# maxsonate/video-diffusion-nnx

Hardware: AMD Instinct MI355X
Metric: denoised frames/sec, 16fx64x64 1000-step DDPM (higher is better)
Workload: dtype bf16; 1 GPU; config_v2_2 (north-star shape): Unet3D dim=64 C=1, 16f x 64x64, DDPM T=1000 p_sample_loop (UNet forward + p_sample per step, hipGraph replay); value = n_gpus*B*F/(T*s_per_step); batch_per_gpu=64, parallelism=dp1 (independent samples, no collective), mfma_operands=bf16, storage=weights fp32 master, activations bf16, fp32 accumulate, process_group=none (single process)

## Files before the change

video_diffusion_nnx_amd/csrc/sla.hip:

```cpp
#include "vdx_common.h"
#include "vdx_internal.h"
#include <stdlib.h>

namespace vdx {

constexpr int SLA_PART = 32 * 32 + 64;

template <int MODE>
__global__ __launch_bounds__(256) void sla_ctx_kernel(const SlaArgs P) {
    using M = Mma<MODE>;
    constexpr int KT = M::KT, KC = M::KC, RS = ROW_STRIDE;
    constexpr int APIECES = KT / 4;
    constexpr int NCHN = 64 / KC;
    constexpr int RSE = NCHN * 64 + 16;

    extern __shared__ __attribute__((aligned(16))) char smem[];
    float* m_run = reinterpret_cast<float*>(smem);
    float* s_run = m_run + 32;
    float* alpha = s_run + 32;
    float* pm = alpha + 32;
    char* xs = smem + 1024;
    char* ws = xs + 64 * RS;
    char* eT = ws + 64 * RS;
    char* vT = eT + 32 * RSE;
// ... 301 lines not shown
#pragma unroll
    for (int tmo = 0; tmo < TMO; ++tmo) {
        const int co = (w * TMO + tmo) * 16 + 4 * q;
        if (co >= P.C) continue;
#pragma unroll
        for (int tn = 0; tn < 4; ++tn) {
            const int row = r0 + tn * 16 + lp;
            if (row >= P.N) continue;
            const float4 xr = load4_f32_or_bf16(P.x, xbase + (size_t)row * P.C + co, P.io_bf16);
            float4 v;
            v.x = oacc[tmo][tn][0] + xr.x; v.y = oacc[tmo][tn][1] + xr.y;
            v.z = oacc[tmo][tn][2] + xr.z; v.w = oacc[tmo][tn][3] + xr.w;
            store4_f32_or_bf16(P.y, xbase + (size_t)row * P.C + co, v, P.io_bf16);
        }
    }
}


template <int MODE, int NKT, bool IO16>
struct SlaTile {
    using M = Mma<MODE>;
    static_assert(!IO16 || MODE == MODE_BF16, "bf16 activation storage implies bf16 MFMA operands");
    static constexpr int PCH = IO16 ? 8 : 4;
    static constexpr int APIECES = M::KT / PCH;
    static constexpr int XP = 64 * APIECES * NKT / 512;
    static constexpr int PLANE = 64 * ROW_STRIDE;
    static constexpr int BUF = NKT * PLANE;
    float4 xpre[XP];
    __device__ __forceinline__ void fetch(const float* x, size_t xbase, int io_bf16, int r0, int N, int C, int tid) {
#pragma unroll
        for (int u = 0; u < XP; ++u) {
            const int i = tid + 512 * u;
            const int kt = i / (64 * APIECES), rem = i % (64 * APIECES);
            const int row = rem / APIECES, c = kt * M::KT + (rem % APIECES) * PCH;
            xpre[u] = make_float4(0.f, 0.f, 0.f, 0.f);
            if (r0 + row < N && c < C) {
                if (IO16) xpre[u] = *reinterpret_cast<const float4*>(reinterpret_cast<const char*>(x) + (xbase + (size_t)(r0 + row) * C + c) * 2);
                else xpre[u] = load4_f32_or_bf16(x, xbase + (size_t)(r0 + row) * C + c, io_bf16);
            }
        }
    }
    __device__ __forceinline__ void put(char* xs, int tid) const {
#pragma unroll
        for (int u = 0; u < XP; ++u) {
            const int i = tid + 512 * u;
            const int kt = i / (64 * APIECES), rem = i % (64 * APIECES);
            char* dst = xs + kt * PLANE + (rem / APIECES) * ROW_STRIDE;
            if (IO16) *reinterpret_cast<float4*>(dst + (rem % APIECES) * 16) = xpre[u];
            else M::store4(dst, (rem % APIECES) * 4, xpre[u]);
        }
    }
};

template <bool FULL>
__device__ __forceinline__ void ctx8_softmax_step(f32x4 (&acc)[2][4], float (&m_run)[2], float (&s_run)[2], f32x4 (&cacc)[2][2], int nleft) {
    constexpr float L2E = 1.44269504088896f;
#pragma unroll
    for (int dt = 0; dt < 2; ++dt) {
        if (!FULL) {
#pragma unroll
            for (int tn = 0; tn < 2; ++tn)
#pragma unroll
                for (int r = 0; r < 4; ++r) if (tn * 16 + r >= nleft) acc[tn][dt][r] = -1e30f;
        }
        float mx = fmaxf(fmaxf(fmaxf(acc[0][dt][0], acc[0][dt][1]), fmaxf(acc[0][dt][2], acc[0][dt][3])),
                         fmaxf(fmaxf(acc[1][dt][0], acc[1][dt][1]), fmaxf(acc[1][dt][2], acc[1][dt][3])));
        mx = max_q(mx);
        const float mn = fmaxf(m_run[dt], mx);
        const float alpha = __builtin_amdgcn_exp2f((m_run[dt] - mn) * L2E);
        m_run[dt] = mn;
        const float nb = -mn * L2E;
        float ssum = 0.f;
#pragma unroll
        for (int tn = 0; tn < 2; ++tn)
#pragma unroll
            for (int r = 0; r < 4; ++r) {
                float e = __builtin_amdgcn_exp2f(__builtin_fmaf(acc[tn][dt][r], L2E, nb));
                if (!FULL) e = (tn * 16 + r >= nleft) ? 0.f : e;
                acc[tn][dt][r] = e;
                ssum += e;
            }
        s_run[dt] = s_run[dt] * alpha + reduce_q(ssum);
#pragma unroll
        for (int et = 0; et < 2; ++et)
#pragma unroll
            for (int r = 0; r < 4; ++r) cacc[et][dt][r] *= alpha;
    }
}

template <int MODE, int NKT, bool IO16>
__global__ __launch_bounds__(512) void sla_ctx8_kernel(const SlaArgs P) {
    using M = Mma<MODE>;
    using T = SlaTile<MODE, NKT, IO16>;
    constexpr int RS = ROW_STRIDE;
    extern __shared__ __attribute__((aligned(16))) char smem[];
    const int tid = threadIdx.x, lane = tid & 63, h = tid >> 6;
    const int lp = lane & 15, q = lane >> 4;
    const int n = blockIdx.x / P.nchunk, chunk = blockIdx.x % P.nchunk;
    const int R = P.nsub * 64;
    const size_t xbase = (size_t)n * P.N * P.C;

    uint4 wf[NKT][2][4];
#pragma unroll
    for (int kt = 0; kt < NKT; ++kt)
#pragma unroll
        for (int ch = 0; ch < 2; ++ch)
#pragma unroll
            for (int tm = 0; tm < 4; ++tm) {
                const char* base = reinterpret_cast<const char*>(tm < 2 ? P.wk : P.wv);
                wf[kt][ch][tm] = *reinterpret_cast<const uint4*>(base + ((size_t)(h * 32 + (tm & 1) * 16 + lp) * P.CPad + kt * M::KT) * M::ES + ch * 64 + q * 16);
            }
    float m_run[2] = {-1e30f, -1e30f}, s_run[2] = {0.f, 0.f};
    f32x4 cacc[2][2];
#pragma unroll
    for (int i = 0; i < 2; ++i) { cacc[i][0] = f32x4{0.f, 0.f, 0.f, 0.f}; cacc[i][1] = f32x4{0.f, 0.f, 0.f, 0.f}; }

    T t;
    t.fetch(P.x, xbase, P.io_bf16, chunk * R, P.N, P.C, tid);
    t.put(smem, tid);
    __syncthreads();
    for (int sub = 0; sub < P.nsub; ++sub) {
        const int r0 = chunk * R + sub * 64;
        if (r0 >= P.N) break;
        const char* xs = smem + (sub & 1) * T::BUF;
        const bool more = (sub + 1 < P.nsub) && (r0 + 64 < P.N);
        if (more) t.fetch(P.x, xbase, P.io_bf16, r0 + 64, P.N, P.C, tid);
#pragma unroll
        for (int hf = 0; hf < 2; ++hf) {
            f32x4 acc[2][4];
#pragma unroll
            for (int i = 0; i < 2; ++i)
#pragma unroll
                for (int j = 0; j < 4; ++j) acc[i][j] = f32x4{0.f, 0.f, 0.f, 0.f};
#pragma unroll
            for (int kt = 0; kt < NKT; ++kt)
#pragma unroll
                for (int ch = 0; ch < 2; ++ch) {
                    uint4 xa[2];
#pragma unroll
                    for (int tn = 0; tn < 2; ++tn)
                        xa[tn] = *reinterpret_cast<const uint4*>(xs + kt * T::PLANE + ((hf * 2 + tn) * 16 + lp) * RS + ch * 64 + q * 16);
#pragma unroll
                    for (int tn = 0; tn < 2; ++tn)
#pragma unroll
                        for (int tm = 0; tm < 4; ++tm) M::mma(acc[tn][tm], xa[tn], wf[kt][ch][tm]);
                }
            if (r0 + 64 <= P.N) ctx8_softmax_step<true>(acc, m_run, s_run, cacc, 0);
            else ctx8_softmax_step<false>(acc, m_run, s_run, cacc, P.N - (r0 + hf * 32 + 4 * q));
#pragma unroll
            for (int tn = 0; tn < 2; ++tn)
#pragma unroll
                for (int et = 0; et < 2; ++et)
#pragma unroll
                    for (int dt = 0; dt < 2; ++dt) M::mma16(cacc[et][dt], acc[tn][2 + et], acc[tn][dt]);
        }
        if (more) t.put(smem + ((sub + 1) & 1) * T::BUF, tid);
        __syncthreads();
    }
    if (P.nchunk == 1) {
        char* ct = reinterpret_cast<char*>(P.ctxT) + (size_t)(n * P.heads + h) * 32 * 32 * M::ES;
#pragma unroll
        for (int dt = 0; dt < 2; ++dt) {
            const float inv = 1.0f / s_run[dt];
#pragma unroll
            for (int et = 0; et < 2; ++et)
#pragma unroll
                for (int r = 0; r < 4; ++r) M::store1(ct + (size_t)(et * 16 + 4 * q + r) * 32 * M::ES, dt * 16 + lp, cacc[et][dt][r] * inv);
        }
        return;
    }
    float* part = P.part + ((size_t)(n * P.nchunk + chunk) * P.heads + h) * SLA_PART;
#pragma unroll
    for (int et = 0; et < 2; ++et)
#pragma unroll
        for (int dt = 0; dt < 2; ++dt)
            *reinterpret_cast<float4*>(part + (dt * 16 + lp) * 32 + et * 16 + 4 * q) =
                make_float4(cacc[et][dt][0], cacc[et][dt][1], cacc[et][dt][2], cacc[et][dt][3]);
    if (q == 0) {
#pragma unroll
        for (int dt = 0; dt < 2; ++dt) { part[1024 + dt * 16 + lp] = m_run[dt]; part[1056 + dt * 16 + lp] = s_run[dt]; }
    }
}

template <int MODE, int NKT, int TMO, int TNO, bool IO16>
__global__ __launch_bounds__(512, NKT == 1 ? 4 : 2) void sla_out8_kernel(const SlaArgs P) {
    using M = Mma<MODE>;
    using T = SlaTile<MODE, NKT, IO16>;
    constexpr int RS = ROW_STRIDE, KC = M::KC, HD = 256;
    constexpr int RSO = HD * M::ES + 16;
    constexpr int NCHO = HD / KC;
    constexpr bool WO_RES = (TMO * NCHO <= 16);

    extern __shared__ __attribute__((aligned(16))) char smem[];
    char* os = smem + 2 * T::BUF;
    constexpr int RSY = NKT * M::KT * 4 + 16;
    char* ys = os + 64 * RSO;
    const int tid = threadIdx.x, lane = tid & 63, h = tid >> 6;
    const int lp = lane & 15, q = lane >> 4;
    const int n = blockIdx.x / P.nchunk, chunk = blockIdx.x % P.nchunk;
    const int R = P.nsub * 64;
    const size_t xbase = (size_t)n * P.N * P.C;

    uint4 wqf[NKT][2][2];
#pragma unroll
    for (int kt = 0; kt < NKT; ++kt)
#pragma unroll
        for (int ch = 0; ch < 2; ++ch)
#pragma unroll
            for (int tm = 0; tm < 2; ++tm)
                wqf[kt][ch][tm] = *reinterpret_cast<const uint4*>(reinterpret_cast<const char*>(P.wq) +
                    ((size_t)(h * 32 + tm * 16 + lp) * P.CPad + kt * M::KT) * M::ES + ch * 64 + q * 16);
// ... 634 lines not shown
```

video_diffusion_nnx_amd/csrc/conv_igemm.hip:

```cpp
#include "vdx_common.h"
#include <type_traits>
#include "vdx_internal.h"
#include "vdx_glds.h"
#include "model.h"
#include <stdlib.h>
#include <string.h>

namespace vdx {

typedef unsigned u32x4 __attribute__((ext_vector_type(4)));
typedef unsigned u32x2 __attribute__((ext_vector_type(2)));
constexpr unsigned OOB = 0xFFFFFFF0u;

template <int MODE, int BC, int TN, int NW, int INF>
__global__ __launch_bounds__(64 * NW, (NW == 8 && TN == 2) ? 4 : 2) void conv_igemm_kernel(const ConvArgs P) {
    using M = Mma<MODE>;
    constexpr int KT = M::KT;
    constexpr int RS = ROW_STRIDE;
    constexpr int WAVES_C = BC / 64;
    constexpr int WAVES_P = NW / WAVES_C;
    constexpr int NT = 64 * NW;
    constexpr int TM = 4;
    constexpr int APIECES = KT / 4;
    constexpr int WREGS = BC * 8 / NT;
// ... 1354 lines not shown
    const int taps = a.kind ? 16 : a.kh * a.kw;
    const double ho = a.kind ? 2.0 * a.H : (a.H + a.stride - 1) / a.stride, wo = a.kind ? 2.0 * a.W : (a.W + a.stride - 1) / a.stride;
    const double cin = a.C0 + a.C1;
    w.flops = 2.0 * a.NF * ho * wo * cin * a.Cout * (a.kind ? 4 : taps);
    w.bytes = (double)a.NF * a.H * a.W * (a.C0 * (a.x0_bf16 ? 2.0 : 4.0) + a.C1 * (a.x1_bf16 ? 2.0 : 4.0)) + a.NF * ho * wo * a.Cout * (a.y_bf16 ? 2.0 : 4.0)
            + (a.res ? a.NF * ho * wo * a.Cout * (a.res_bf16 ? 2.0 : 4.0) : 0.0) + es * taps * cin * a.Cout;
    snprintf(w.shape, sizeof(w.shape), "%s%dx%d %d->%d %dx%dx%d%s%s%s%s", a.kind ? "convT" : "conv", a.kind ? 4 : a.kh, a.kind ? 4 : a.kw, a.C0 + a.C1, a.Cout,
             a.NF, a.H, a.W, a.stride == 2 ? " s2" : "", a.pro ? " +prologue" : "", a.res ? " +res" : "", a.C1 ? " concat" : "");
    return w;
}
}

static bool tiles16_3x3(int mode, const ConvArgs& a) {
    return mode == MODE_BF16 && a.kind == 0 && a.kh == 3 && a.kw == 3 && a.stride == 1 && a.H % 16 == 0 && a.W % 16 == 0 &&
           (long)a.NF * (a.H / 16) * (a.W / 16) >= 1024;
}
static bool conv64_shape(int mode, const ConvArgs& a) {
    return tiles16_3x3(mode, a) && a.C0 == 64 && a.C1 == 0 && a.Cout == 64 && a.wrows >= 64 && a.wrow0 >= 0 && a.wrow0 + 64 <= a.wrows &&
           (!a.res || (!a.pro && a.x0_bf16 && !a.res_bf16)) && (size_t)a.NF * a.H * a.W * 64 * (a.y_bf16 ? 2 : 4) < 0xFFFFFFF0ull &&
           (!a.pro || (a.groups <= 32 && 64 % a.groups == 0)) && (!a.out_stats || (a.out_groups <= 32 && 64 % a.out_groups == 0));
}
static bool conv64q_pro_eligible(int mode, const ConvArgs& a) { return conv64_shape(mode, a) && a.x0_bf16 && a.pro; }
static bool conv64r_eligible(int mode, const ConvArgs& a) { return conv64_shape(mode, a) && a.x0_bf16 && !a.pro && !a.res; }
static bool conv64d_eligible(int mode, const ConvArgs& a) { return conv64_shape(mode, a) && a.x0_bf16 && !a.pro && a.res; }
static bool conv64p_eligible(int mode, const ConvArgs& a) { return conv64_shape(mode, a) && !a.x0_bf16; }
static bool conv64p_c32_eligible(int mode, const ConvArgs& a) {
    return tiles16_3x3(mode, a) && a.C0 == 32 && a.C1 == 0 && a.Cout == 32 && a.wrows == 32 && a.wrow0 == 0 && a.CinPad == 64 && a.x0_bf16 &&
           a.y_bf16 && !a.res && (!a.pro || (a.groups <= 32 && 32 % a.groups == 0)) && (!a.out_stats || (a.out_groups <= 32 && 32 % a.out_groups == 0));
}
static bool conv64q_cout32_eligible(int mode, const ConvArgs& a) {
    return tiles16_3x3(mode, a) && a.Cout == 32 && a.x0_bf16 && a.x1_bf16 && !a.pro && a.y_bf16 && ((a.C0 == 32 && a.C1 == 32) || (a.C0 == 64 && a.C1 == 64)) &&
           a.CinPad == a.C0 + a.C1 && a.wrows == 32 && a.wrow0 == 0 && !a.res &&
           (!a.out_stats || (a.out_groups <= 32 && 32 % a.out_groups == 0 && (32 / a.out_groups) <= 8 && 8 % (32 / a.out_groups) == 0));
}
static bool conv64q_cin128_eligible(int mode, const ConvArgs& a) {
    return tiles16_3x3(mode, a) && a.Cout == 64 && a.x0_bf16 && (!a.C1 || a.x1_bf16) && !a.pro && ((a.C0 == 64 && a.C1 == 64) || (a.C0 == 128 && a.C1 == 0)) &&
           a.wrows == 64 && a.wrow0 == 0 && !a.res && (!a.out_stats || (a.out_groups <= 32 && 32 % (64 / a.out_groups) == 0 && 64 % a.out_groups == 0)) &&
           (long)a.NF * a.H * a.W * 256 < 0xFFFFFFF0l;
}

hipError_t launch_conv(int mode, ConvArgs a, hipStream_t st) {
    const int K = a.kind ? 2 : a.kh;
    if (a.kind) { a.stride = 1; a.Ho = a.H; a.Wo = a.W; a.Hy = 2 * a.H; a.Wy = 2 * a.W; }
    else { a.Ho = (a.H + a.stride - 1) / a.stride; a.Wo = (a.W + a.stride - 1) / a.stride; a.Hy = a.Ho; a.Wy = a.Wo; }
    a.CinPad = conv_cin_pad(mode, a.C0 + a.C1);
    const int ES = mode == MODE_F32 ? 4 : 2;
    const size_t npix = (size_t)a.NF * a.H * a.W;
    if (a.wrows <= 0) { a.wrows = a.Cout; a.wrow0 = 0; }
    const size_t b0 = npix * a.C0 * (a.x0_bf16 ? 2 : 4), b1 = npix * a.C1 * (a.x1_bf16 ? 2 : 4), bw = (size_t)(a.kind ? 16 : a.kh * a.kw) * a.wrows * a.CinPad * ES;
    if (b0 >= 0xFFFFFFF0ull || b1 >= 0xFFFFFFF0ull || bw >= 0xFFFFFFF0ull) return hipErrorInvalidValue;
    a.x0_bytes = (unsigned)b0; a.x1_bytes = (unsigned)b1; a.w_bytes = (unsigned)bw;
    if (conv3x3_ws_eligible(mode, a)) {
        const ConvWork cw = conv_work(mode, a);
        LaunchScope ls(st, "conv3x3_ws_kernel", cw.flops, cw.bytes, "<%d, %s> %s", conv3x3_ws_geo(a), a.pro ? "true" : "false", cw.shape);
        return launch_conv3x3_ws(a, st);
    }
    if (conv4x4_ws_eligible(mode, a)) {
        const ConvWork cw = conv_work(mode, a);
        LaunchScope ls(st, "conv4x4_ws_kernel", cw.flops, cw.bytes, "<%d, %d, %d> %s", a.kind == 1 ? a.H : a.H / 2, a.kind == 1 ? 2 : 1, a.Cout == 64 ? 64 : 128, cw.shape);
        return launch_conv4x4_ws(a, st);
    }
    if (resample32_eligible(mode, a)) {
        const ConvWork cw = conv_work(mode, a);
        LaunchScope ls(st, "resample32_kernel", cw.flops, cw.bytes, "<%d> %s", a.kind, cw.shape);
        return launch_resample32(a, st);
    }
    if (conv1x1_pw_eligible(mode, a)) {
        const ConvWork cw = conv_work(mode, a);
        LaunchScope ls(st, "conv1x1_pw_kernel", cw.flops, cw.bytes, "<%d> %s", conv1x1_pw_rows(a), cw.shape);
        return launch_conv1x1_pw(a, st);
    }
    if (conv64q_pro_eligible(mode, a)) {
        const ConvWork cw = conv_work(mode, a);
        LaunchScope ls(st, "conv64q_kernel", cw.flops, cw.bytes, "<cin 64, pro %d, y16 %d> %s", a.pro, a.y_bf16, cw.shape);
        return launch_conv64q(a, st);
    }
    if (conv64r_eligible(mode, a)) {
        const ConvWork cw = conv_work(mode, a);
        LaunchScope ls(st, "conv64r_kernel", cw.flops, cw.bytes, "<pro 0, y16 %d> %s", a.y_bf16, cw.shape);
        return launch_conv64r(a, st);
    }
    if (conv64d_eligible(mode, a)) {
        const ConvWork cw = conv_work(mode, a);
        LaunchScope ls(st, "conv64d_kernel", cw.flops, cw.bytes, "<x16 %d, pro %d, y16 %d, res %d> %s", a.x0_bf16, a.pro, a.y_bf16, a.res ? 1 : 0, cw.shape);
        return launch_conv64d(a, st);
    }
    if (conv64p_eligible(mode, a)) {
        const ConvWork cw = conv_work(mode, a);
        LaunchScope ls(st, "conv64p_kernel", cw.flops, cw.bytes, "<x16 %d, pro %d, y16 %d, res %d> %s", a.x0_bf16, a.pro, a.y_bf16, a.res ? 1 : 0, cw.shape);
        return launch_conv64p(a, st);
    }
    if (conv64p_c32_eligible(mode, a)) {
        const ConvWork cw = conv_work(mode, a);
        LaunchScope ls(st, "conv64p_kernel", cw.flops, cw.bytes, "<x16 1, pro %d, y16 1, res 0, C 32> %s", a.pro, cw.shape);
        return launch_conv64p(a, st);
    }
    if (conv64q_cout32_eligible(mode, a)) {
        const ConvWork cw = conv_work(mode, a);
        LaunchScope ls(st, "conv64q_kernel", cw.flops, cw.bytes, "<cin %d, pro 0, y16 1, cout 32> %s", a.C0 + a.C1, cw.shape);
        return launch_conv64q(a, st);
    }
    if (conv64q_cin128_eligible(mode, a)) {
        const ConvWork cw = conv_work(mode, a);
        LaunchScope ls(st, "conv64q_kernel", cw.flops, cw.bytes, "<cin 128, pro 0, y16 %d> %s", a.y_bf16, cw.shape);
        return launch_conv64q(a, st);
    }
    const int BC = a.Cout <= 64 ? 64 : 128;
// ... 46 lines not shown
```

video_diffusion_nnx_amd/csrc/conv_ws.hip:

```cpp
#include "vdx_common.h"
#include "vdx_internal.h"
#include "vdx_glds.h"
#include <type_traits>

namespace vdx {

namespace {

__device__ __attribute__((aligned(16))) unsigned g_zero_page[4];

__device__ __forceinline__ int frag_off(int row, int key, int q) { return row * 128 + (((q ^ (key & 3)) | (key & 4)) << 4); }

constexpr int WS_SLAB = 128 * 128;
constexpr int WS_STORES = 16;

}

constexpr int WS_NS = 4;

template <int GEO> struct WsGeo {
    static constexpr bool WF = GEO != 0;
    static constexpr int S = WF ? GEO : 16;
    static constexpr int NP = WF ? 256 / (S * S) : 1;
    static constexpr int IW = 18;
// ... 265 lines not shown
        hbuf ^= 1;
    };

    bool after_epilogue = false;
    for (int t = t0; t < t1; ++t) {
#pragma unroll
        for (int tm = 0; tm < 4; ++tm)
#pragma unroll
            for (int tn = 0; tn < 4; ++tn) acc[tm][tn] = f32x4{0.f, 0.f, 0.f, 0.f};
        for (int cc = 0; cc < nchunks; ++cc) {
            const bool last = (cc + 1 == nchunks);
            const bool more = !last || (t + 1 < t1);
            const int tnext = last ? (t + 1 < t1 ? t + 1 : t) : t, ccnext = last ? 0 : cc + 1;
            if (PRO && more) {
                const int bn = sample_of(tnext);
                if (bn != bcoef) { make_coef(bn); bcoef = bn; }
            }
            if (after_epilogue) run_chunk(std::true_type{}, tnext, ccnext, more);
            else run_chunk(std::false_type{}, tnext, ccnext, more);
            after_epilogue = false;
        }
        {
            const int b = sample_of(t);
            if (b != bcur) { flush_stats(bcur); bcur = b; }
            size_t tile_pix;
            int nrows = 256;
            if (WF) { tile_pix = wf_pix0(t); nrows = wf_rows(t); }
            else { const int f = t / tiles_pf, rem = t - f * tiles_pf, ty = rem / tiles_x, tx = rem - ty * tiles_x;
                   tile_pix = ((size_t)f * P.H + (size_t)ty * 16) * P.W + (size_t)tx * 16; }
            const int cobase = j * 128 + wc * 64 + 4 * q;
#pragma unroll
            for (int tm = 0; tm < 4; ++tm) {
                float s = 0.f, ss = 0.f;
                const float4 bs = *reinterpret_cast<const float4*>(biasl + wc * 64 + tm * 16 + 4 * q);
#pragma unroll
                for (int tn = 0; tn < 4; ++tn) {
                    if (WF && opix[tn] >= nrows) continue;
                    const float4 v = make_float4(acc[tm][tn][0] + bs.x, acc[tm][tn][1] + bs.y, acc[tm][tn][2] + bs.z, acc[tm][tn][3] + bs.w);
                    const size_t e = (tile_pix + opix[tn]) * P.Cout + cobase + tm * 16;
                    if (P.y_bf16) *reinterpret_cast<uint2*>(reinterpret_cast<char*>(P.y) + e * 2) = make_uint2(pack_bf16x2(v.x, v.y), pack_bf16x2(v.z, v.w));
                    else *reinterpret_cast<float4*>(P.y + e) = v;
                    s += (v.x + v.y) + (v.z + v.w);
                    ss += (v.x * v.x + v.y * v.y) + (v.z * v.z + v.w * v.w);
                }
                st_s[tm] += s; st_q[tm] += ss;
            }
            after_epilogue = true;
        }
    }
    flush_stats(bcur);
    wait_vm_lgkm0<0>();
}

template <int GEO, int KIND, int BCO>
__global__ __launch_bounds__(512, 2) void conv4x4_ws_kernel(const ConvArgs P, const int tiles_per_range, const int total_vtiles, const int nct) {
    using M = Mma<MODE_BF16>;
    static_assert((GEO == 8 || GEO == 16 || GEO == 32) && (KIND == 1 || KIND == 2) && (BCO == 64 || BCO == 128), "geometry");
    constexpr bool BAND = GEO == 32;
    constexpr int S = GEO;
    constexpr int NP = BAND ? 1 : 256 / (S * S);
    constexpr int ZROW = BAND ? 320 : 256;
    constexpr int HPX = ZROW + 1, NPIECE = HPX * 8, NU = (NPIECE + 511) / 512, NUMIN = NPIECE / 512, HBUF = HPX * 128;
    constexpr int NS = WS_NS;
    constexpr int WIN = BCO / 64;
    constexpr int SLAB = BCO * 128;
    constexpr int TN = BCO == 128 ? 4 : 2;
    constexpr int STORES = 4 * TN;

    extern __shared__ __attribute__((aligned(16))) char smem[];
    char* ring = smem;
    char* halo = ring + NS * SLAB;
    float* biasl = reinterpret_cast<float*>(halo + 2 * HBUF);
    const unsigned ring_a = lds_addr(ring), halo_a = lds_addr(halo);
    const int tid = threadIdx.x, lane = tid & 63;
    const int wave = __builtin_amdgcn_readfirstlane(tid >> 6);
    const int r = lane & 15, q = lane >> 4;
    const int wc = BCO == 128 ? (wave & 1) : 0, wpx = BCO == 128 ? (wave >> 1) : wave;
    const int xcd = blockIdx.x & 7, slot = blockIdx.x >> 3;
    const int j = slot % nct;
    const int range = (slot / nct) * 8 + xcd;
    const int t0 = range * tiles_per_range, t1 = min(t0 + tiles_per_range, total_vtiles);
    if (t0 >= t1) return;
    const int C = P.C0;
    const int ncc = C >> 6;
    const int nchunks = KIND == 1 ? 4 * ncc : ncc;

    unsigned wsrc[WIN];
#pragma unroll
    for (int v = 0; v < WIN; ++v) {
        const int i2 = (v * 8 + wave) * 64 + lane, row = i2 >> 3, pos = i2 & 7;
        wsrc[v] = (unsigned)((j * BCO + row) * P.CinPad) * 2u + (unsigned)((pos ^ (row & 7)) << 4);
    }
    const size_t tap_stride = (size_t)P.Cout * P.CinPad * 2;
    const char* wbase = reinterpret_cast<const char*>(P.wp);
    auto piece = [&](int u, int l, int& row, int& chunk) -> bool {
        const int i = (u * 8 + wave) * 64 + l;
        row = i >> 3;
        chunk = (i & 7) ^ (row & 7);
        return i < NPIECE;
    };
    auto opaque_lane = [&]() { int l = lane; asm volatile("" : "+v"(l)); return l; };
    const char* const zero_page = reinterpret_cast<const char*>(g_zero_page);
    constexpr int DYB = S * 128;
    const int halo_o = NS * SLAB;
    const int aoff = frag_off(wc * 64 + r, r, q);
    int b3[TN][3], zs[3], opix[TN];
// ... 180 lines not shown
    if (a.C0 % 64 || (a.Cout % 128 && a.Cout != 64) || a.CinPad != a.C0) return false;
    const int nct = a.Cout == 64 ? 1 : a.Cout / 128;
    if (nct != 1 && nct != 2 && nct != 4 && nct != 8) return false;
    if (a.wrows != a.Cout || a.wrow0 != 0) return false;
    const long vtiles = (long)a.NF * geo * geo / 256 * (a.kind == 1 ? 4 : 1);
    if (vtiles * nct < 128) return false;
    if ((size_t)a.NF * a.H * a.W * (size_t)a.C0 * 2 >= 0xFFFF0000ull || (size_t)a.NF * 4 * geo * geo >= 0x7FFFFFFFull) return false;
    return true;
}

hipError_t launch_conv4x4_ws(const ConvArgs& a, hipStream_t st) {
    const int geo = ws4_geo(a), bco = a.Cout == 64 ? 64 : 128, nct = a.Cout / bco, up = a.kind == 1;
    const int total = (int)((long)a.NF * geo * geo / 256) * (up ? 4 : 1);
    const int cus = device_cus();
    const int unit = 8 * nct;
    int grid = std::max(unit, cus / unit * unit);
    grid = std::min(grid, (total * nct + unit - 1) / unit * unit);
    const int nranges = grid / nct;
    int tpr = (total + nranges - 1) / nranges;
    if (up) tpr = (tpr + 3) / 4 * 4;
    const size_t lds = (size_t)WS_NS * bco * 128 + 2 * (size_t)(geo == 32 ? 321 : 257) * 128 + 512;
    auto go = [&](auto kfn) -> hipError_t {
        if (hipError_t e = lds_opt_in(kfn, lds); e != hipSuccess) return e;
        hipLaunchKernelGGL(kfn, dim3(grid), dim3(512), lds, st, a, tpr, total, nct);
        return hipGetLastError();
    };
#define VDX_WS4(G_) do { if (bco == 64) return up ? go(conv4x4_ws_kernel<G_, 2, 64>) : go(conv4x4_ws_kernel<G_, 1, 64>);       \
                         return up ? go(conv4x4_ws_kernel<G_, 2, 128>) : go(conv4x4_ws_kernel<G_, 1, 128>); } while (0)
    if (geo == 8) VDX_WS4(8);
    if (geo == 16) VDX_WS4(16);
    VDX_WS4(32);
#undef VDX_WS4
}

bool conv3x3_ws_eligible(int mode, const ConvArgs& a) {
    if (mode != MODE_BF16 || a.kind != 0 || a.kh != 3 || a.kw != 3 || a.stride != 1 || a.res) return false;
    if (!a.x0_bf16 || (a.C1 && !a.x1_bf16)) return false;
    if (a.C0 % 64 || a.C1 % 64 || a.Cout % 128) return false;
    const int nct = a.Cout / 128;
    if (nct != 1 && nct != 2 && nct != 4 && nct != 8) return false;
    if (a.wrows != a.Cout || a.wrow0 != 0) return false;
    const int geo = ws_geo(a);
    if (geo < 0) return false;
    if (geo != 0 && (a.F <= 0 || a.NF % a.F)) return false;
    if (a.pro && (a.C1 || a.groups < 1 || a.groups > 32 || a.C0 % a.groups || a.C0 > 1024)) return false;
    if (a.out_stats && (a.out_groups < 1 || a.Cout % a.out_groups || (a.Cout / a.out_groups) % 16)) return false;
    const int npf = geo == 0 ? 1 : 256 / (a.H * a.W);
    const long tiles = geo == 0 ? (long)a.NF * (a.H / 16) * (a.W / 16) : (long)(a.NF / a.F) * ((a.F + npf - 1) / npf);
    if (tiles * nct < 128) return false;
    if ((size_t)a.NF * a.H * a.W * (size_t)std::max(a.C0, a.C1) * 2 >= 0xFFFF0000ull) return false;
    return true;
}

hipError_t launch_conv3x3_ws(const ConvArgs& a, hipStream_t st) {
    const int geo = ws_geo(a);
    const int nct = a.Cout / 128;
    const int npf = geo == 0 ? 1 : 256 / (a.H * a.W);
    const int total = geo == 0 ? a.NF * (a.H / 16) * (a.W / 16) : (a.NF / a.F) * ((a.F + npf - 1) / npf);
    const int cus = device_cus();
    const int unit = 8 * nct;
    int grid = std::max(unit, cus / unit * unit);
    grid = std::min(grid, (total * nct + unit - 1) / unit * unit);
    const int nranges = grid / nct;
    const int tpr = (total + nranges - 1) / nranges;
    const int HPX = geo == 0 ? 18 * 18 : 257;
    const size_t lds = (size_t)WS_NS * WS_SLAB + 2 * (size_t)HPX * 128 + 512 + (a.pro ? (size_t)a.CinPad * 8 + 256 : 0);
    if (lds > 160 * 1024) return hipErrorInvalidValue;
    auto go = [&](auto kfn) -> hipError_t {
        if (hipError_t e = lds_opt_in(kfn, lds); e != hipSuccess) return e;
#ifndef VDX_WS_PIN_MB
#define VDX_WS_PIN_MB 0
#endif
        const size_t wbytes = (size_t)9 * a.Cout * a.CinPad * 2;
        const int pin = (VDX_WS_PIN_MB > 0 && nct > 1 && wbytes > (size_t)VDX_WS_PIN_MB * 1024 * 1024) ? 1 : 0;
        hipLaunchKernelGGL(kfn, dim3(grid), dim3(512), lds, st, a, tpr, total, nct, pin);
        return hipGetLastError();
    };
    if (geo == 0) return a.pro ? go(conv3x3_ws_kernel<0, true>) : go(conv3x3_ws_kernel<0, false>);
    if (geo == 8) return a.pro ? go(conv3x3_ws_kernel<8, true>) : go(conv3x3_ws_kernel<8, false>);
    return a.pro ? go(conv3x3_ws_kernel<16, true>) : go(conv3x3_ws_kernel<16, false>);
}

}
```

video_diffusion_nnx_amd/csrc/vdx_internal.h:

```cpp
#pragma once
#include <hip/hip_runtime.h>
#include <stdarg.h>
#include <stddef.h>
#include <stdio.h>
#include <algorithm>
#include "../../include/vdx.h"

int vdx_set_error(int code, const char* msg, const char* file, int line);

namespace vdx {

extern vdx_launch_hook g_launch_hook;
extern void* g_launch_hook_user;
struct LaunchScope {
    vdx_launch_info info; char desc[192]; hipStream_t st; bool on;
    LaunchScope(hipStream_t s, const char* kernel, double flops, double bytes, const char* fmt, ...) __attribute__((format(printf, 6, 7))) : st(s), on(g_launch_hook != nullptr) {
        if (!on) return;
        va_list ap;
        va_start(ap, fmt);
        vsnprintf(desc, sizeof(desc), fmt, ap);
        va_end(ap);
        info.kernel = kernel; info.shape = desc; info.flops = flops; info.bytes = bytes;
        g_launch_hook(g_launch_hook_user, 0, &info, st);
    }
// ... 179 lines not shown
hipError_t launch_norm_bwd(NormBwdArgs a, hipStream_t st);
size_t norm_bwd_scratch_floats(int C, int batch, long pix_per_sample);

struct AttnBwdArgs {
    const float* qkv; const float* dO; float* O; float* dq; float* dk; float* dv;
    int heads, L; long nseq, inner, outer_p, tok_p; float scale;
    int dstride;
    int io_bf16;
    int bf16_mma;
};
hipError_t launch_attn_core_bwd(const AttnBwdArgs& a, hipStream_t st);
struct AttnBwdXArgs {
    const float* x; const float* g;
    int x_bf16;
    const void* wqkv; const float* bqkv;
    const void* woT;
    void* O; void* dqkv;
    float* dx;
    int L; long nseq, inner, outer_p, tok_p; float scale;
};
hipError_t launch_attn_bwd_fused(const AttnBwdXArgs& a, hipStream_t st);
struct SlaBwdArgs {
    const float* q; const float* k; const float* v; const float* dOut; float* O; float* dq; float* dk; float* dv; float* A;
    int NF, N, heads;
    int dstride;
    int io_bf16;
    int bf16_mma;
};
size_t sla_bwd_scratch_floats(int NF, int heads);
hipError_t launch_sla_bwd(const SlaBwdArgs& a, hipStream_t st);

hipError_t launch_final_conv_bwd(const float* x, const float* dout, const float* w, float* dx, float* dW, float* db, long npix, int D, int Cout, int x_bf16, hipStream_t st, float* part = nullptr, size_t part_cap = 0);
hipError_t launch_init_conv_wgrad(const float* x, const float* dy, float* dW, float* db, int B, int Cin, int F, int H, int W, int Cout, int K, hipStream_t st, float* part = nullptr, size_t part_cap = 0);
hipError_t launch_resblock_ss_bwd(const float* params, float* grads, const float* temb, const SsLayer* layers, int nlayers, const float* lin_base,
                                  float* dss_base, float* dtemb, int temb_dim, int B, hipStream_t st, float* part = nullptr, size_t part_cap = 0);
hipError_t launch_time_mlp_bwd(const TimeMlpArgs& a, const float* dtemb, float* dw1, float* db1, float* dw2, float* db2, float* dnull, int B, hipStream_t st);

size_t conv_packed_bytes(int mode, int taps, int Cin, int Cout);
int conv_cin_pad(int mode, int Cin);
hipError_t launch_pack_weights(int mode, const float* src, void* dst, int taps, int Cin, int Cout, hipStream_t st);
hipError_t launch_conv(int mode, ConvArgs a, hipStream_t st);
int conv3x3_ws_geo(const ConvArgs& a);
bool conv4x4_ws_eligible(int mode, const ConvArgs& a);
hipError_t launch_conv4x4_ws(const ConvArgs& a, hipStream_t st);
hipError_t launch_gn_silu_apply16(float* y_bf16, const double* stats, const float* gamma, const float* beta, const float* ss, int ss_stride, int groups,
                                  int C, int batch, long pix_per_sample, hipStream_t st);
bool resample32_eligible(int mode, const ConvArgs& a);
hipError_t launch_resample32(const ConvArgs& a, hipStream_t st);
bool conv1x1_pw_eligible(int mode, const ConvArgs& a);
hipError_t launch_conv1x1_pw(const ConvArgs& a, hipStream_t st);
int conv1x1_pw_rows(const ConvArgs& a);
bool conv3x3_ws_eligible(int mode, const ConvArgs& a);
hipError_t launch_conv3x3_ws(const ConvArgs& a, hipStream_t st);
hipError_t launch_pack_weights_t(int mode, const float* src, void* dst, int taps, int Cin, int Cout, hipStream_t st);

}
```

Measured before the change: 48.64 frames/s.

## Use lazy max rescaling and MFMA row-sums in SLA context softmax

Restructures the sla_ctx8 online-softmax loop. Exponentials are computed against a stale running max, and the max update plus rescale happen only when some exponent exceeds a bound, in which case the keys are recomputed. Row sums move from shuffle reductions to an MFMA against a ones vector, and the subtile width becomes configurable (TNS, default 1) with an occupancy hint in launch_bounds. The aim is to cut per-tile max and reduction work and register pressure in this attention kernel. The cost is possible re-projection on the slow path and looser numeric bounds on the exponentials.

```diff
diff --git a/video_diffusion_nnx_amd/csrc/sla.hip b/video_diffusion_nnx_amd/csrc/sla.hip
--- a/video_diffusion_nnx_amd/csrc/sla.hip
+++ b/video_diffusion_nnx_amd/csrc/sla.hip
@@ -377,35 +377,82 @@
     }
 };
 
+#ifndef CTX8_TNS
+#define CTX8_TNS 1
+#endif
+constexpr int TNS = CTX8_TNS;
+
+template <int MODE, int NKT, int TM0, int TM1>
+__device__ __forceinline__ void ctx8_project(f32x4 (&acc)[TNS][4], const char* xs, const uint4 (&wf)[NKT][2][4], int st, int lp, int q) {
+    using M = Mma<MODE>;
+    constexpr int PLANE = 64 * ROW_STRIDE;
+#pragma unroll
+    for (int tn = 0; tn < TNS; ++tn)
+#pragma unroll
+        for (int tm = TM0; tm < TM1; ++tm) acc[tn][tm] = f32x4{0.f, 0.f, 0.f, 0.f};
+#pragma unroll
+    for (int kt = 0; kt < NKT; ++kt)
+#pragma unroll
+        for (int ch = 0; ch < 2; ++ch) {
+            uint4 xa[TNS];
+#pragma unroll
+            for (int tn = 0; tn < TNS; ++tn)
+                xa[tn] = *reinterpret_cast<const uint4*>(xs + kt * PLANE + ((st * TNS + tn) * 16 + lp) * ROW_STRIDE + ch * 64 + q * 16);
+#pragma unroll
+            for (int tn = 0; tn < TNS; ++tn)
+#pragma unroll
+                for (int tm = TM0; tm < TM1; ++tm) M::mma(acc[tn][tm], xa[tn], wf[kt][ch][tm]);
+        }
+}
+
+constexpr float CTX8_LAZY_BOUND = 256.f;
+constexpr float CTX8_L2E = 1.44269504088896f;
+
 template <bool FULL>
-__device__ __forceinline__ void ctx8_softmax_step(f32x4 (&acc)[2][4], float (&m_run)[2], float (&s_run)[2], f32x4 (&cacc)[2][2], int nleft) {
-    constexpr float L2E = 1.44269504088896f;
+__device__ __forceinline__ float ctx8_exp_lazy(f32x4 (&acc)[TNS][4], const float (&nb)[2], int nleft) {
+    float mx = 0.f;
+#pragma unroll
+    for (int dt = 0; dt < 2; ++dt)
+#pragma unroll
+        for (int tn = 0; tn < TNS; ++tn)
+#pragma unroll
+            for (int r = 0; r < 4; ++r) {
+                float e = __builtin_amdgcn_exp2f(__builtin_fmaf(acc[tn][dt][r], CTX8_L2E, nb[dt]));
+                if (!FULL) e = (tn * 16 + r >= nleft) ? 0.f : e;
+                acc[tn][dt][r] = e;
+                mx = fmaxf(mx, e);
+            }
+    return mx;
+}
+
+template <bool FULL>
+__device__ __forceinline__ void ctx8_softmax_step(f32x4 (&acc)[TNS][4], float (&m_run)[2], f32x4 (&sacc)[2], f32x4 (&cacc)[2][2], int nleft) {
 #pragma unroll
     for (int dt = 0; dt < 2; ++dt) {
         if (!FULL) {
 #pragma unroll
-            for (int tn = 0; tn < 2; ++tn)
+            for (int tn = 0; tn < TNS; ++tn)
 #pragma unroll
                 for (int r = 0; r < 4; ++r) if (tn * 16 + r >= nleft) acc[tn][dt][r] = -1e30f;
         }
-        float mx = fmaxf(fmaxf(fmaxf(acc[0][dt][0], acc[0][dt][1]), fmaxf(acc[0][dt][2], acc[0][dt][3])),
-                         fmaxf(fmaxf(acc[1][dt][0], acc[1][dt][1]), fmaxf(acc[1][dt][2], acc[1][dt][3])));
+        float mx = -1e30f;
+#pragma unroll
+        for (int tn = 0; tn < TNS; ++tn) mx = fmaxf(mx, fmaxf(fmaxf(acc[tn][dt][0], acc[tn][dt][1]), fmaxf(acc[tn][dt][2], acc[tn][dt][3])));
         mx = max_q(mx);
         const float mn = fmaxf(m_run[dt], mx);
-        const float alpha = __builtin_amdgcn_exp2f((m_run[dt] - mn) * L2E);
+        const float alpha = __builtin_amdgcn_exp2f((m_run[dt] - mn) * CTX8_L2E);
         m_run[dt] = mn;
-        const float nb = -mn * L2E;
-        float ssum = 0.f;
-#pragma unroll
-        for (int tn = 0; tn < 2; ++tn)
+        const float nb = -mn * CTX8_L2E;
+#pragma unroll
+        for (int tn = 0; tn < TNS; ++tn)
 #pragma unroll
             for (int r = 0; r < 4; ++r) {
-                float e = __builtin_amdgcn_exp2f(__builtin_fmaf(acc[tn][dt][r], L2E, nb));
+                float e = __builtin_amdgcn_exp2f(__builtin_fmaf(acc[tn][dt][r], CTX8_L2E, nb));
                 if (!FULL) e = (tn * 16 + r >= nleft) ? 0.f : e;
                 acc[tn][dt][r] = e;
-                ssum += e;
-            }
-        s_run[dt] = s_run[dt] * alpha + reduce_q(ssum);
+            }
+#pragma unroll
+        for (int r = 0; r < 4; ++r) sacc[dt][r] *= alpha;
 #pragma unroll
         for (int et = 0; et < 2; ++et)
 #pragma unroll
@@ -414,10 +461,9 @@
 }
 
 template <int MODE, int NKT, bool IO16>
-__global__ __launch_bounds__(512) void sla_ctx8_kernel(const SlaArgs P) {
+__global__ __launch_bounds__(512, NKT == 1 ? 4 : 2) void sla_ctx8_kernel(const SlaArgs P) {
     using M = Mma<MODE>;
     using T = SlaTile<MODE, NKT, IO16>;
-    constexpr int RS = ROW_STRIDE;
     extern __shared__ __attribute__((aligned(16))) char smem[];
     const int tid = threadIdx.x, lane = tid & 63, h = tid >> 6;
     const int lp = lane & 15, q = lane >> 4;
@@ -435,10 +481,12 @@
                 const char* base = reinterpret_cast<const char*>(tm < 2 ? P.wk : P.wv);
                 wf[kt][ch][tm] = *reinterpret_cast<const uint4*>(base + ((size_t)(h * 32 + (tm & 1) * 16 + lp) * P.CPad + kt * M::KT) * M::ES + ch * 64 + q * 16);
             }
-    float m_run[2] = {-1e30f, -1e30f}, s_run[2] = {0.f, 0.f};
+    float m_run[2] = {-1e30f, -1e30f}, nb[2] = {1e30f * CTX8_L2E, 1e30f * CTX8_L2E};
     f32x4 cacc[2][2];
-#pragma unroll
-    for (int i = 0; i < 2; ++i) { cacc[i][0] = f32x4{0.f, 0.f, 0.f, 0.f}; cacc[i][1] = f32x4{0.f, 0.f, 0.f, 0.f}; }
+    f32x4 sacc[2];
+    const f32x4 ones = f32x4{1.f, 1.f, 1.f, 1.f};
+#pragma unroll
+    for (int i = 0; i < 2; ++i) { cacc[i][0] = f32x4{0.f, 0.f, 0.f, 0.f}; cacc[i][1] = f32x4{0.f, 0.f, 0.f, 0.f}; sacc[i] = f32x4{0.f, 0.f, 0.f, 0.f}; }
 
     T t;
     t.fetch(P.x, xbase, P.io_bf16, chunk * R, P.N, P.C, tid);
@@ -449,39 +497,35 @@
         if (r0 >= P.N) break;
         const char* xs = smem + (sub & 1) * T::BUF;
         const bool more = (sub + 1 < P.nsub) && (r0 + 64 < P.N);
+        const bool full = r0 + 64 <= P.N;
         if (more) t.fetch(P.x, xbase, P.io_bf16, r0 + 64, P.N, P.C, tid);
 #pragma unroll
-        for (int hf = 0; hf < 2; ++hf) {
-            f32x4 acc[2][4];
-#pragma unroll
-            for (int i = 0; i < 2; ++i)
-#pragma unroll
-                for (int j = 0; j < 4; ++j) acc[i][j] = f32x4{0.f, 0.f, 0.f, 0.f};
-#pragma unroll
-            for (int kt = 0; kt < NKT; ++kt)
-#pragma unroll
-                for (int ch = 0; ch < 2; ++ch) {
-                    uint4 xa[2];
-#pragma unroll
-                    for (int tn = 0; tn < 2; ++tn)
-                        xa[tn] = *reinterpret_cast<const uint4*>(xs + kt * T::PLANE + ((hf * 2 + tn) * 16 + lp) * RS + ch * 64 + q * 16);
-#pragma unroll
-                    for (int tn = 0; tn < 2; ++tn)
-#pragma unroll
-                        for (int tm = 0; tm < 4; ++tm) M::mma(acc[tn][tm], xa[tn], wf[kt][ch][tm]);
-                }
-            if (r0 + 64 <= P.N) ctx8_softmax_step<true>(acc, m_run, s_run, cacc, 0);
-            else ctx8_softmax_step<false>(acc, m_run, s_run, cacc, P.N - (r0 + hf * 32 + 4 * q));
-#pragma unroll
-            for (int tn = 0; tn < 2; ++tn)
+        for (int st = 0; st < 4 / TNS; ++st) {
+            f32x4 acc[TNS][4];
+            ctx8_project<MODE, NKT, 0, 4>(acc, xs, wf, st, lp, q);
+            const int nleft = P.N - (r0 + st * TNS * 16 + 4 * q);
+            const float emax = full ? ctx8_exp_lazy<true>(acc, nb, 0) : ctx8_exp_lazy<false>(acc, nb, nleft);
+            if (__builtin_amdgcn_ballot_w64(emax > CTX8_LAZY_BOUND) != 0) {
+                ctx8_project<MODE, NKT, 0, 2>(acc, xs, wf, st, lp, q);
+                if (full) ctx8_softmax_step<true>(acc, m_run, sacc, cacc, 0);
+                else ctx8_softmax_step<false>(acc, m_run, sacc, cacc, nleft);
+                nb[0] = -m_run[0] * CTX8_L2E; nb[1] = -m_run[1] * CTX8_L2E;
+            }
+#pragma unroll
+            for (int tn = 0; tn < TNS; ++tn)
 #pragma unroll
                 for (int et = 0; et < 2; ++et)
 #pragma unroll
                     for (int dt = 0; dt < 2; ++dt) M::mma16(cacc[et][dt], acc[tn][2 + et], acc[tn][dt]);
+#pragma unroll
+            for (int tn = 0; tn < TNS; ++tn)
+#pragma unroll
+                for (int dt = 0; dt < 2; ++dt) M::mma16(sacc[dt], ones, acc[tn][dt]);
         }
         if (more) t.put(smem + ((sub + 1) & 1) * T::BUF, tid);
         __syncthreads();
     }
+    const float s_run[2] = {sacc[0][0], sacc[1][0]};
     if (P.nchunk == 1) {
         char* ct = reinterpret_cast<char*>(P.ctxT) + (size_t)(n * P.heads + h) * 32 * 32 * M::ES;
 #pragma unroll
```

Result: no change. 49.05 frames/s, median of 6 (+0.8%).

## Add 256-output-channel weight-streaming 3x3 conv kernel using 32x32x16 MFMA

Applied to the files above, without the earlier changes.

Adds a new variant of the weight-streaming 3x3 conv kernel for whole-frame geometries (8x8 and 16x16) that tiles 256 output channels per block instead of 128. It uses 32x32x16 bf16 MFMA, a 5-deep weight ring and double-buffered halo, and is dispatched whenever Cout is a multiple of 256 and no GroupNorm prologue is fused. The aim is to double reuse of each halo/activation load across output channels and raise MFMA efficiency on the small-spatial, wide-channel layers. In exchange it uses more LDS and registers per block, and the grid has fewer blocks, which could hurt occupancy or load balance.

```diff
diff --git a/video_diffusion_nnx_amd/csrc/conv_igemm.hip b/video_diffusion_nnx_amd/csrc/conv_igemm.hip
--- a/video_diffusion_nnx_amd/csrc/conv_igemm.hip
+++ b/video_diffusion_nnx_amd/csrc/conv_igemm.hip
@@ -1430,7 +1430,8 @@
     a.x0_bytes = (unsigned)b0; a.x1_bytes = (unsigned)b1; a.w_bytes = (unsigned)bw;
     if (conv3x3_ws_eligible(mode, a)) {
         const ConvWork cw = conv_work(mode, a);
-        LaunchScope ls(st, "conv3x3_ws_kernel", cw.flops, cw.bytes, "<%d, %s> %s", conv3x3_ws_geo(a), a.pro ? "true" : "false", cw.shape);
+        LaunchScope ls(st, "conv3x3_ws_kernel", cw.flops, cw.bytes, "<%d, %s%s> %s", conv3x3_ws_geo(a), a.pro ? "true" : "false",
+                       conv3x3_ws_co256(a) ? ", co256" : "", cw.shape);
         return launch_conv3x3_ws(a, st);
     }
     if (conv4x4_ws_eligible(mode, a)) {
diff --git a/video_diffusion_nnx_amd/csrc/conv_ws.hip b/video_diffusion_nnx_amd/csrc/conv_ws.hip
--- a/video_diffusion_nnx_amd/csrc/conv_ws.hip
+++ b/video_diffusion_nnx_amd/csrc/conv_ws.hip
@@ -341,6 +341,230 @@
     wait_vm_lgkm0<0>();
 }
 
+constexpr int WS2_NS = 5;
+constexpr int WS2_HSLAB = 256 * 64;
+typedef float f32x16 __attribute__((ext_vector_type(16)));
+
+template <int GEO>
+__global__ __launch_bounds__(512, 2) void conv3x3_ws256_kernel(const ConvArgs P, const int tiles_per_range, const int total_tiles, const int nct) {
+    static_assert(GEO == 8 || GEO == 16, "whole frames only");
+    constexpr int S = GEO, NP = 256 / (S * S);
+    constexpr int HPX = 257, NPIECE = HPX * 8, NU = (NPIECE + 511) / 512, NUMIN = NPIECE / 512, HBUF = HPX * 128;
+    constexpr int NS = WS2_NS;
+    constexpr int WIN = 4;
+    constexpr int DYB = S * 128;
+
+    extern __shared__ __attribute__((aligned(16))) char smem[];
+    char* ring = smem;
+    char* halo = ring + NS * WS2_HSLAB;
+    float* biasl = reinterpret_cast<float*>(halo + 2 * HBUF);
+    const unsigned ring_a = lds_addr(ring), halo_a = lds_addr(halo);
+    const int tid = threadIdx.x, lane = tid & 63;
+    const int wave = __builtin_amdgcn_readfirstlane(tid >> 6);
+    const int n = lane & 31, hl = lane >> 5;
+    const int wc = wave & 1, wpx = wave >> 1;
+    const int xcd = blockIdx.x & 7, slot = blockIdx.x >> 3;
+    const int j = slot % nct;
+    const int range = (slot / nct) * 8 + xcd;
+    const int t0 = range * tiles_per_range, t1 = min(t0 + tiles_per_range, total_tiles);
+    if (t0 >= t1) return;
+    const int nchunks = P.CinPad >> 6;
+    const int tps = (P.F + NP - 1) / NP;
+    auto sample_of = [&](int t) { return t / tps; };
+    auto wf_pix0 = [&](int t) { const int b = t / tps, k = t - b * tps; return (unsigned)(b * P.F + k * NP) * (unsigned)(S * S); };
+    auto wf_rows = [&](int t) { const int k = t % tps; return min(NP, P.F - k * NP) * (S * S); };
+
+    unsigned wsrc[2];
+#pragma unroll
+    for (int v = 0; v < 2; ++v) {
+        const int i2 = (v * 8 + wave) * 64 + lane, row = i2 >> 2, pos = i2 & 3;
+        wsrc[v] = (unsigned)((j * 256 + row) * P.CinPad) * 2u + (unsigned)((pos ^ ((row >> 2) & 3)) << 4);
+    }
+    const size_t tap_stride = (size_t)P.Cout * P.CinPad * 2;
+    const char* wbase = reinterpret_cast<const char*>(P.wp);
+    auto piece = [&](int u, int l, int& row, int& chunk) -> bool {
+        const int i = (u * 8 + wave) * 64 + l;
+        row = i >> 3;
+        chunk = (i & 7) ^ ((row >> 1) & 7);
+        return i < NPIECE;
+    };
+    auto opaque_lane = [&]() { int l = lane; asm volatile("" : "+v"(l)); return l; };
+    const char* const zero_page = reinterpret_cast<const char*>(g_zero_page);
+    const int halo_o = NS * WS2_HSLAB;
+    const int aoff = (wc * 128 + n) * 64 + ((hl ^ ((n >> 2) & 3)) << 4);
+    int b3[2][3], zs[3];
+#pragma unroll
+    for (int tn = 0; tn < 2; ++tn) {
+        const int p = wpx * 64 + tn * 32 + n;
+#pragma unroll
+        for (int dx = 0; dx < 3; ++dx) {
+            const int r0 = p - S - 1 + dx;
+            b3[tn][dx] = halo_o + r0 * 128 + ((hl ^ ((r0 >> 1) & 7)) << 4);
+        }
+    }
+#pragma unroll
+    for (int dy = 0; dy < 3; ++dy) zs[dy] = halo_o + 256 * 128 - dy * DYB;
+    auto tap_valid = [&](int tn, int dy, int dx) -> bool {
+        const int p = wpx * 64 + tn * 32 + n, y = (p / S) % S + dy - 1, x = p % S + dx - 1;
+        return y >= 0 && y < S && x >= 0 && x < S;
+    };
+    if (tid < 256) biasl[tid] = P.bias ? P.bias[j * 256 + tid] : 0.f;
+
+    int pcc = 0, ptap = 0, ph = 0, pslot = 0;
+    auto issue_w = [&]() {
+        const char* src = wbase + (size_t)ptap * tap_stride + (size_t)((pcc << 7) + (ph << 6));
+        const unsigned dst = __builtin_amdgcn_readfirstlane(ring_a + pslot * WS2_HSLAB + wave * 1024);
+        glds16(src + wsrc[0], dst);
+        glds16(src + wsrc[1], dst + 8 * 1024);
+        if (++ph == 2) { ph = 0; if (++ptap == 9) { ptap = 0; if (++pcc == nchunks) pcc = 0; } }
+        if (++pslot == NS) pslot = 0;
+    };
+    auto issue_halo = [&](int t, int cc, int buf) {
+        const bool second = (cc << 6) >= P.C0;
+        const char* xb = reinterpret_cast<const char*>(second ? P.x1 : P.x0);
+        const int Cs = second ? P.C1 : P.C0, cb = (cc << 6) - (second ? P.C0 : 0);
+        const unsigned dst = __builtin_amdgcn_readfirstlane(halo_a + buf * HBUF + wave * 1024);
+        const int l = opaque_lane();
+        const unsigned pix0 = wf_pix0(t);
+        const int nrows = wf_rows(t);
+#pragma unroll
+        for (int u = 0; u < NU; ++u) {
+            int row, ch;
+            if (piece(u, l, row, ch)) {
+                const bool ok = row < nrows;
+                const unsigned off = ((pix0 + row) * Cs + cb + (ch << 3)) * 2u;
+                const void* src = ok ? static_cast<const void*>(xb + off) : static_cast<const void*>(zero_page);
+                glds16(src, dst + u * 8 * 1024);
+            }
+        }
+    };
+    float st_s[4] = {0.f, 0.f, 0.f, 0.f}, st_q[4] = {0.f, 0.f, 0.f, 0.f};
+    auto flush_stats = [&](int b) {
+        if (!P.out_stats) return;
+        const int cpg = P.Cout / P.out_groups;
+#pragma unroll
+        for (int tm = 0; tm < 4; ++tm) {
+            const float s1 = reduce_q(reduce16(st_s[tm])), s2 = reduce_q(reduce16(st_q[tm]));
+            st_s[tm] = 0.f; st_q[tm] = 0.f;
+            if (lane == 0) {
+                const int g = (j * 256 + wc * 128 + tm * 32) / cpg;
+                double* dst = P.out_stats + (((size_t)b * GN_SLOTS + ((blockIdx.x + wave) % GN_SLOTS)) * P.out_groups + g) * 2;
+                unsafeAtomicAdd(dst, (double)s1); unsafeAtomicAdd(dst + 1, (double)s2);
+            }
+        }
+    };
+    auto ldA = [&](uint4 (&a)[4], int sl, int s) {
+        const int base = (sl * WS2_HSLAB + aoff) ^ (s * 32);
+#pragma unroll
+        for (int tm = 0; tm < 4; ++tm) a[tm] = *reinterpret_cast<const uint4*>(ring + base + tm * 2048);
+    };
+    auto ldB = [&](uint4 (&b)[2], int tap, int h, int s) {
+        const int dy = tap / 3, dx = tap - 3 * dy;
+        const int X = (h * 64 + s * 32) ^ ((S == 8 && dy == 1) ? 64 : 0);
+#pragma unroll
+        for (int tn = 0; tn < 2; ++tn) {
+            int a = tap_valid(tn, dy, dx) ? b3[tn][dx] : zs[dy];
+            asm volatile("" : "+v"(a));
+            b[tn] = *reinterpret_cast<const uint4*>(smem + ((a ^ X) + dy * DYB));
+        }
+    };
+    auto mma = [](f32x16& c, const uint4& a, const uint4& b) {
+        c = __builtin_amdgcn_mfma_f32_32x32x16_bf16(__builtin_bit_cast(bf16x8, a), __builtin_bit_cast(bf16x8, b), c, 0, 0, 0);
+    };
+    auto flip_buffers = [&](int to_buf1) {
+        const int d = to_buf1 ? HBUF : -HBUF;
+#pragma unroll
+        for (int tn = 0; tn < 2; ++tn)
+#pragma unroll
+            for (int dx = 0; dx < 3; ++dx) b3[tn][dx] += d;
+#pragma unroll
+        for (int dy = 0; dy < 3; ++dy) zs[dy] += d;
+    };
+
+    issue_halo(t0, 0, 0);
+#pragma unroll
+    for (int k = 0; k < NS - 1; ++k) issue_w();
+    wait_vm_lgkm0<0>();
+    __builtin_amdgcn_s_barrier();
+
+    int cslot = 0, hbuf = 0, bcur = sample_of(t0);
+    f32x16 acc[4][2];
+    uint4 pa[4], pb[2];
+    ldA(pa, 0, 0); ldB(pb, 0, 0, 0);
+    auto run_chunk = [&](int tnext, int ccnext) {
+#pragma unroll
+        for (int k = 0; k < 18; ++k) {
+            const int tap = k >> 1, h = k & 1;
+            if (k == 0) wait_vm<WIN>();
+            else if (k < 3) wait_vm<WIN + NUMIN>();
+            else wait_vm<WIN>();
+            __builtin_amdgcn_s_barrier();
+            if (k == 0) issue_halo(tnext, ccnext, hbuf ^ 1);
+            issue_w();
+            uint4 a1[4], b1[2];
+            ldA(a1, cslot, 1); ldB(b1, tap, h, 1);
+#pragma unroll
+            for (int tm = 0; tm < 4; ++tm)
+#pragma unroll
+                for (int tn = 0; tn < 2; ++tn) mma(acc[tm][tn], pa[tm], pb[tn]);
+            const int nslot = (cslot + 1 == NS) ? 0 : cslot + 1;
+            if (k == 17) flip_buffers(hbuf ^ 1);
+            ldA(pa, nslot, 0);
+            ldB(pb, k == 17 ? 0 : (k + 1) >> 1, k == 17 ? 0 : (k + 1) & 1, 0);
+#pragma unroll
+            for (int tm = 0; tm < 4; ++tm)
+#pragma unroll
+                for (int tn = 0; tn < 2; ++tn) mma(acc[tm][tn], a1[tm], b1[tn]);
+            cslot = nslot;
+        }
+        hbuf ^= 1;
+    };
+
+    for (int t = t0; t < t1; ++t) {
+#pragma unroll
+        for (int tm = 0; tm < 4; ++tm)
+#pragma unroll
+            for (int tn = 0; tn < 2; ++tn) acc[tm][tn] = f32x16{};
+        for (int cc = 0; cc < nchunks; ++cc) {
+            const bool last = (cc + 1 == nchunks);
+            const int tnext = last ? (t + 1 < t1 ? t + 1 : t) : t, ccnext = last ? 0 : cc + 1;
+            run_chunk(tnext, ccnext);
+        }
+        {
+            const int b = sample_of(t);
+            if (b != bcur) { flush_stats(bcur); bcur = b; }
+            const int nrows = wf_rows(t);
+            const int l = opaque_lane();
+            const int co = wc * 128 + 4 * (l >> 5);
+            char* const ytile = reinterpret_cast<char*>(P.y) + ((size_t)wf_pix0(t) * P.Cout + j * 256 + co) * (P.y_bf16 ? 2 : 4);
+#pragma unroll
+            for (int tm = 0; tm < 4; ++tm) {
+                float s = 0.f, ss = 0.f;
+#pragma unroll
+                for (int tn = 0; tn < 2; ++tn) {
+                    const int p = wpx * 64 + tn * 32 + (l & 31);
+                    if (p >= nrows) continue;
+#pragma unroll
+                    for (int g = 0; g < 4; ++g) {
+                        const float4 bs = *reinterpret_cast<const float4*>(biasl + co + tm * 32 + 8 * g);
+                        const f32x16& c = acc[tm][tn];
+                        const float4 v = make_float4(c[4 * g] + bs.x, c[4 * g + 1] + bs.y, c[4 * g + 2] + bs.z, c[4 * g + 3] + bs.w);
+                        const unsigned e = (unsigned)p * P.Cout + tm * 32 + 8 * g;
+                        if (P.y_bf16) *reinterpret_cast<uint2*>(ytile + e * 2) = make_uint2(pack_bf16x2(v.x, v.y), pack_bf16x2(v.z, v.w));
+                        else *reinterpret_cast<float4*>(ytile + e * 4) = v;
+                        s += (v.x + v.y) + (v.z + v.w);
+                        ss += (v.x * v.x + v.y * v.y) + (v.z * v.z + v.w * v.w);
+                    }
+                }
+                st_s[tm] += s; st_q[tm] += ss;
+            }
+            wait_vm<0>();
+        }
+    }
+    flush_stats(bcur);
+    wait_vm_lgkm0<0>();
+}
+
 template <int GEO, int KIND, int BCO>
 __global__ __launch_bounds__(512, 2) void conv4x4_ws_kernel(const ConvArgs P, const int tiles_per_range, const int total_vtiles, const int nct) {
     using M = Mma<MODE_BF16>;
@@ -627,8 +851,32 @@
     return true;
 }
 
+bool conv3x3_ws_co256(const ConvArgs& a) {
+    const int geo = ws_geo(a);
+    if ((geo != 8 && geo != 16) || a.pro || a.Cout % 256) return false;
+    if (a.out_stats && (a.Cout / a.out_groups) % 32) return false;
+    return true;
+}
+
 hipError_t launch_conv3x3_ws(const ConvArgs& a, hipStream_t st) {
     const int geo = ws_geo(a);
+    if (conv3x3_ws_co256(a)) {
+        const int nct = a.Cout / 256;
+        const int total = (a.NF / a.F) * ((a.F + 256 / (geo * geo) - 1) / (256 / (geo * geo)));
+        const int cus = device_cus();
+        const int unit = 8 * nct;
+        int grid = std::max(unit, cus / unit * unit);
+        grid = std::min(grid, (total * nct + unit - 1) / unit * unit);
+        const int nranges = grid / nct;
+        const int tpr = (total + nranges - 1) / nranges;
+        const size_t lds = (size_t)WS2_NS * WS2_HSLAB + 2 * (size_t)257 * 128 + 256 * 4;
+        auto go = [&](auto kfn) -> hipError_t {
+            if (hipError_t e = lds_opt_in(kfn, lds); e != hipSuccess) return e;
+            hipLaunchKernelGGL(kfn, dim3(grid), dim3(512), lds, st, a, tpr, total, nct);
+            return hipGetLastError();
+        };
+        return geo == 8 ? go(conv3x3_ws256_kernel<8>) : go(conv3x3_ws256_kernel<16>);
+    }
     const int nct = a.Cout / 128;
     const int npf = geo == 0 ? 1 : 256 / (a.H * a.W);
     const int total = geo == 0 ? a.NF * (a.H / 16) * (a.W / 16) : (a.NF / a.F) * ((a.F + npf - 1) / npf);
diff --git a/video_diffusion_nnx_amd/csrc/vdx_internal.h b/video_diffusion_nnx_amd/csrc/vdx_internal.h
--- a/video_diffusion_nnx_amd/csrc/vdx_internal.h
+++ b/video_diffusion_nnx_amd/csrc/vdx_internal.h
@@ -255,6 +255,7 @@
 int conv1x1_pw_rows(const ConvArgs& a);
 bool conv3x3_ws_eligible(int mode, const ConvArgs& a);
 hipError_t launch_conv3x3_ws(const ConvArgs& a, hipStream_t st);
+bool conv3x3_ws_co256(const ConvArgs& a);
 hipError_t launch_pack_weights_t(int mode, const float* src, void* dst, int taps, int Cin, int Cout, hipStream_t st);
 
 }
```

Measured after the change: 48.42 frames/s before, 48.76 frames/s after, median of 6. No clear change (+0.7%).
